# tiborcamargo/KinectPy

Hardware: AMD Instinct MI355X
Metric: Mpoints/sec end-to-end (unproject+filter+ICP), 4-sensor frame (higher is better)
Workload: dtype f64 decisions / f32 storage

## Files before the change

kinectpy_amd/csrc/kpx_icpiter.h:

```cpp
#pragma once
#include "kpx_icpdefs.h"
#include "kpx_fixed.h"
#include "kpx_icpsolve.h"
#include "kpx_nnlocal.h"

namespace kpx {

constexpr int kIRows = kIWaves * kLRows;
constexpr int kCertHist = 64;
constexpr int kChainRec = 32;
constexpr int kChainRecords = 64;
constexpr int kChainWords = 24;
constexpr unsigned long long kChainEmpty = 0xFFF8C0DEC0DEC0DEull;
constexpr int kAccSet = kAccCopies * kAcc * kFixedWords;
constexpr int kStampBlocks = 4096;
__device__ unsigned long long g_icp_stamp[kStampBlocks][8];
__device__ unsigned long long g_icp_wave[kStampBlocks * 4][4];
__device__ unsigned long long g_cert_check[8];
__device__ unsigned long long g_chain_stamp[64][48];
__device__ __forceinline__ void chain_tick(unsigned long long *row, int slot, bool on)
{
    if (row && on) row[slot] = wall_clock64();
}
__device__ __forceinline__ void phase_tick(unsigned long long *__restrict__ armed, int slot, unsigned bid)
{
    if (!armed || threadIdx.x || bid >= kStampBlocks) return;
    __builtin_nontemporal_store(wall_clock64(), &g_icp_stamp[bid][slot]);
}
__device__ __forceinline__ double cert_skin(bool certs, int k, const IcpState *st, double max_d2, const CertPolicy &pol)
{
    double c_skin = 0.0;
    if (certs && k > 0) {
        const double lm = st->last_motion, md = sqrt(max_d2);
        if (lm <= (double)pol.calm * md) c_skin = fmin(fmax((double)pol.factor * lm, (double)pol.smin * md), (double)pol.smax * md);
    }
    return c_skin;
}
__device__ __forceinline__ bool cert_test(const double s[3], const float src[3], int32_t prev, const float pt[3], int32_t bj, uint32_t cert, const double *Th,
                                          double c_reach, double c_skin, int cert_check, double &rb0)
{
    double d1 = c_reach;
    if (bj != INT_MAX) {
        const double dx = s[0] - (double)pt[0], dy = s[1] - (double)pt[1], dz = s[2] - (double)pt[2];
        d1 = sqrt(fma(dz, dz, fma(dy, dy, dx * dx))) * (1.0 + 1e-12);
    }
    const bool keeps = (prev >= 0) == (bj != INT_MAX);
    const float Lc = __uint_as_float(cert & ~63u);
    double pc[3] = { 0.0, 0.0, 0.0 };
    if (Lc > 0.0f) {
        const double x = src[0], y = src[1], z = src[2];
#pragma unroll
        for (int a = 0; a < 3; ++a) pc[a] = fma(Th[4 * a], x, fma(Th[4 * a + 1], y, fma(Th[4 * a + 2], z, Th[4 * a + 3])));
    }
    const double ex = s[0] - pc[0], ey = s[1] - pc[1], ez = s[2] - pc[2];
    const double moved = sqrt(fma(ez, ez, fma(ey, ey, ex * ex))) * (1.0 + 1e-12);
    const bool certd = Lc > 0.0f && keeps && (d1 + moved) * (1.0 + 1e-6) + 1e-6 < (double)Lc;
    if (certd && !cert_check) rb0 = -1.0;
    else if (c_skin > 0.0) { const double rr = d1 + c_skin; rb0 = fmax(rb0, rr * rr); }
    return certd;
}
__device__ __forceinline__ uint32_t cert_word(unsigned sec, double eps_out, double rb_out, int k)
{
    typedef unsigned uu2 __attribute__((ext_vector_type(2)));
    const uu2 pat = { 0u, sec };
    const double d2nd = sec == 0xFFFFFFFFu ? INFINITY : __builtin_bit_cast(double, pat) - 1.0 - eps_out;
    const double l2 = fmin(rb_out, d2nd);
    const uint32_t lb = l2 > 0.0 && k < kCertHist ? (__float_as_uint(f32_down(sqrt(l2) * (1.0 - 1e-7))) & ~63u) : 0u;
    return lb > 63u ? (lb | (uint32_t)k) : 0u;
}
__device__ __forceinline__ void cert_check_disagreement(int k, int64_t row, int32_t kept, int32_t found, uint32_t word)
{
    if (atomicAdd(&g_cert_check[2], 1ull) == 0ull) {
        g_cert_check[3] = (unsigned long long)k; g_cert_check[4] = (unsigned long long)row;
        g_cert_check[5] = (unsigned long long)(unsigned)kept; g_cert_check[6] = (unsigned long long)(unsigned)found;
        g_cert_check[7] = (unsigned long long)(word & ~63u);
    }
}
__device__ __forceinline__ void cert_check_count(bool first, int k, const IcpState *st, double c_skin, int certified, int searched)
{
    if (first && g_cert_check[2] == 0ull) {
        g_cert_check[3] = (unsigned long long)k; g_cert_check[4] = __builtin_bit_cast(unsigned long long, st->last_motion);
        g_cert_check[5] = __builtin_bit_cast(unsigned long long, st->motion); g_cert_check[6] = __builtin_bit_cast(unsigned long long, c_skin);
    }
    atomicAdd(&g_cert_check[0], (unsigned long long)certified);
    atomicAdd(&g_cert_check[1], (unsigned long long)searched);
}
__device__ __forceinline__ IcpFuse ticket_fuse(const IcpProblem &P, int max_iter, double rel_fit, double rel_rmse, unsigned long long tag, int light,
                                               CertPolicy pol, double *chain_rec, unsigned long long *stamp)
{
    return IcpFuse{ (IcpState *)nullptr, P.ring, max_iter, rel_fit, rel_rmse, P.result, P.progress, tag, P.ring + kAccSet,
                    (light & 1) ? P.light_key : (double *)nullptr, P.sbbox, (light & 2) ? P.cert : (uint32_t *)nullptr,
                    (light & 2) ? P.thist : (double *)nullptr, (light & 4) ? 1 : 0, pol, chain_rec, stamp };
}
template <int THREADS, bool SEARCHED>
__device__ __forceinline__ unsigned long long winner_take(unsigned long long *acc, unsigned long long *ticket, bool plane, double *s_sums, int tix_w)
{
    if (tix_w < kAcc) s_sums[tix_w] = acc_live(plane, tix_w) ? fixed_total_coherent(acc, tix_w) : 0.0;
    const unsigned long long n_searched = SEARCHED ? searched_take(ticket, tix_w) : 0ull;
    if (THREADS > 64) __syncthreads(); else wave_lds_fence();
    for (int e = tix_w; e < kAccSet; e += THREADS) __hip_atomic_store(acc + e, 0ull, __ATOMIC_RELAXED, __HIP_MEMORY_SCOPE_AGENT);
    if (tix_w == 0) __hip_atomic_store(ticket, 0ull, __ATOMIC_RELAXED, __HIP_MEMORY_SCOPE_AGENT);
    return n_searched;
}
__device__ __forceinline__ void winner_publish(IcpState *st, const IcpState *work, double *thist, int k, unsigned long long *progress, unsigned long long tag,
                                               unsigned long long n_searched, int64_t n, int lane)
{
    if (lane < (int)(sizeof(IcpState) / sizeof(double))) reinterpret_cast<double *>(st)[lane] = reinterpret_cast<const double *>(work)[lane];
    if (thist && k + 1 < kCertHist && lane < 12) thist[12 * (k + 1) + lane] = work->T[lane];
    if (lane == 0 && progress)
        __hip_atomic_store(progress, tag | progress_searched(n_searched, n) | ((unsigned long long)(work->done ? 1 : 0) << 32) | (unsigned long long)(unsigned)(k + 1),
                           __ATOMIC_RELAXED, __HIP_MEMORY_SCOPE_SYSTEM);
}

template <bool PERSIST = false>
__device__ __forceinline__ void icp_iter_body(const unsigned bid, const unsigned nblocks, const float *__restrict__ src, int64_t n, const float *__restrict__ tgt,
                                                       const float *__restrict__ tn, const double *__restrict__ Bs,
                                                       const int32_t *__restrict__ orig, const float *__restrict__ tile_box,
                                                       const float *__restrict__ group_box, int32_t n_groups,
                                                       const double *__restrict__ tbbox, const int32_t *__restrict__ row_of,
                                                       const float *__restrict__ src_sorted, int32_t *__restrict__ idx_sorted,
                                                       float *__restrict__ ptgt_sorted,
                                                       int32_t *__restrict__ idx_cur, double *__restrict__ d2_cur, double max_d2, int mode,
                                                       int k, const IcpState *__restrict__ st, unsigned long long *acc,
                                                       unsigned long long *__restrict__ tile_visits, IcpFuse fuse)
{
    const unsigned tix = PERSIST ? (unsigned)opaque_i((int)threadIdx.x) : threadIdx.x;
    __shared__ IcpState s_state;
    __shared__ double s_sums[kAcc];
    __shared__ float rowk[kIWaves][16][8];
    __shared__ float rowsrc[kIWaves][16][3];
    __shared__ uint32_t rowc[kIWaves][16];
    __shared__ int32_t rowi[kIWaves][16][2];
    __shared__ double s_key;
    const int wave = PERSIST ? __builtin_amdgcn_readfirstlane((int)(tix >> 6)) : (int)(tix >> 6), lane = tix & 63, q = lane >> 4, j = lane & 15;
    const int64_t row_base = ((int64_t)bid * kIWaves + wave) * kLRows;
    const int64_t last = n - 1;
    const unsigned long long t_block_start = (tile_visits && tix == 0) ? wall_clock64() : 0ull;
    const double t2max = target_t2max(tbbox);
    float my_src[3] = { 0.0f, 0.0f, 0.0f }, my_pt[3] = { 0.0f, 0.0f, 0.0f }, my_nrm[3] = { 0.0f, 0.0f, 0.0f };
    int32_t my_row = 0, my_prev = -1;
    uint32_t my_cert = 0u;
    const bool certs = fuse.ticket && fuse.light_key && fuse.cert;
    if (PERSIST && k > 0) {
        if (lane < 16) {
            my_row = rowi[wave][lane][1];
#pragma unroll
            for (int a = 0; a < 3; ++a) { my_src[a] = rowsrc[wave][lane][a]; my_pt[a] = rowk[wave][lane][a]; my_nrm[a] = rowk[wave][lane][3 + a]; }
            my_prev = __float_as_int(rowk[wave][lane][6]);
            if (certs) my_cert = rowc[wave][lane];
        }
    } else if (lane < 16) {
        const int64_t r = row_base + lane < last ? row_base + lane : last;
        if (idx_cur || d2_cur) my_row = row_of[r];
#pragma unroll
        for (int a = 0; a < 3; ++a) my_src[a] = src_sorted[3 * r + a];
        if (PERSIST) {
#pragma unroll
            for (int a = 0; a < 3; ++a) rowsrc[wave][lane][a] = my_src[a];
            rowc[wave][lane] = 0u;
        }
        if (k > 0) {
            my_prev = idx_sorted[r];
#pragma unroll
            for (int a = 0; a < 3; ++a) my_pt[a] = ptgt_sorted[3 * r + a];
            if (certs) my_cert = fuse.cert[r];
        }
    }
    __shared__ double s_thist[kCertHist][12];
    if (PERSIST) {
        if (certs && k < kCertHist && tix < 12) s_thist[k][tix] = st->T[tix];
    } else if (certs && k > 0)
        for (int e = tix; e < 12 * (k < kCertHist ? k : kCertHist); e += kIThreads) (&s_thist[0][0])[e] = fuse.thist[e];
    GroupPre gpre;
    group_pre_load(gpre, group_box, n_groups, lane);
    if (!PERSIST && mode == 1 && k > 0 && lane < 16) {
        const float *np_ = tn + 3 * (int64_t)(my_prev > 0 ? my_prev : 0);
#pragma unroll
        for (int a = 0; a < 3; ++a) my_nrm[a] = np_[a];
    }
    const double *Tk = st->T;
    static_assert(sizeof(IcpState) % sizeof(double) == 0, "IcpState is copied as doubles");
    if (fuse.ticket && tix < sizeof(IcpState) / sizeof(double))
        reinterpret_cast<double *>(&s_state)[tix] = reinterpret_cast<const double *>(st)[tix];
    if (fuse.pair) {
        const IcpState *in = fuse.pair + ((k + 1) & 1);
        IcpState *out = fuse.pair + (k & 1);
        const unsigned long long *prev = fuse.ring + (int64_t)((k + 2) % 3) * kAccSet;
        if (k > 0 && tix < kAcc) s_sums[tix] = acc_live(mode == 1, (int)tix) ? fixed_total(prev, tix) : 0.0;
        if (tix == 0) s_state = *in;
        __syncthreads();
        if (s_state.done) {
            if (bid == 0 && tix == 0) *out = s_state;
            return;
        }
        __shared__ FinishScratch s_fs;
        if (k > 0 && wave == 0)
            icp_finish_wave(s_sums, n, mode, k - 1, fuse.max_iter, fuse.rel_fit, fuse.rel_rmse, &s_state, bid == 0 ? fuse.result : (double *)nullptr,
                            s_fs, lane);
        __syncthreads();
        if (bid == 0) {
            unsigned long long *next = fuse.ring + (int64_t)((k + 1) % 3) * kAccSet;
            for (int e = tix; e < kAccSet; e += kIThreads) next[e] = 0ull;
            if (tix == 0) {
                *out = s_state;
                if (k > 0 && fuse.progress)
                    __hip_atomic_store(fuse.progress, fuse.tag | ((unsigned long long)(s_state.done ? 1 : 0) << 32) | (unsigned long long)(unsigned)k,
                                       __ATOMIC_RELEASE, __HIP_MEMORY_SCOPE_SYSTEM);
            }
        }
        if (s_state.done) return;
        Tk = s_state.T;
        acc = fuse.ring + (int64_t)(k % 3) * kAccSet;
    } else if (st->done) return;
    bool skip = false;
    if (fuse.ticket && fuse.light_key) {
        const double key = PERSIST ? (k > 0 ? s_key : 0.0) : fuse.light_key[bid];
        skip = key > 0.0 && (st->motion + st->reach) * (1.0 + 1e-6) + 1e-6 < key;
    }
    __shared__ double s_light[kIWaves];
    const int nacc = mode == 1 ? kAcc : 17;
    if (tile_visits && tix == 0 && bid < kStampBlocks) { g_icp_stamp[bid][7] = skip ? 1ull : 0ull; g_icp_stamp[bid][6] = (unsigned long long)nblocks; }
    do {
    if (skip) break;
    __shared__ int32_t lists[kIWaves][kLScratch];
    __shared__ double rowd[kIWaves][16][kRowStride];
    __shared__ float rowf[kIWaves][16][kRowFStride];
    __shared__ double sh[kAcc][kIRows + 1];
    if (tile_visits && tix == 0 && bid < kStampBlocks) {
        g_icp_stamp[bid][0] = t_block_start;
        g_icp_stamp[bid][6] = (unsigned long long)nblocks;
    }
    phase_tick(tile_visits, 1, bid);
    if (certs && (k > 0 || PERSIST)) __syncthreads();
    if (PERSIST && fuse.stamp && tix == 0) {
        const unsigned long long t = wall_clock64();
        if (bid == 0) fuse.stamp[0] = t;
        atomicMax(&fuse.stamp[5], t);
        atomicMin(&fuse.stamp[10], t);
    }

    const double c_reach = certs ? st->reach : 0.0;
    const double c_skin = cert_skin(certs, k, st, max_d2, fuse.pol);
    bool my_active = true, my_certd = false;
    if (lane < 16) {
        const int64_t i = my_row;
        double s[3];
        xform_row(Tk, my_src, s);
        const double seed = row_seed(s);
        double bv = INFINITY;
        int32_t bj = INT_MAX;
        if (k > 0 && my_prev >= 0) { bv = partner_bound(s, seed, my_pt); bj = my_prev; }
        bound_clamp(seed, max_d2, t2max, bv, bj);
        double rb0 = bv - 1.0;
        if (certs) {
            const bool certd = cert_test(s, my_src, my_prev, my_pt, bj, my_cert, s_thist[my_cert & 63u], c_reach, c_skin, fuse.cert_check, rb0);
            my_active = (!certd || fuse.cert_check) && row_base + lane <= last;
            my_certd = certd && row_base + lane <= last;
        }
        rowd[wave][lane][0] = s[0]; rowd[wave][lane][1] = s[1]; rowd[wave][lane][2] = s[2];
        rowd[wave][lane][3] = rb0;
        rowd[wave][lane][4] = seed; rowd[wave][lane][5] = bv;
        rowi[wave][lane][0] = bj; rowi[wave][lane][1] = (int32_t)i;
#pragma unroll
        for (int a = 0; a < 3; ++a) { rowk[wave][lane][a] = my_pt[a]; rowk[wave][lane][3 + a] = my_nrm[a]; }
        rowk[wave][lane][6] = __int_as_float(my_prev);
    }
    if (PERSIST && fuse.stamp) {
        const bool searched = lane < 16 && my_active && !my_certd;
        const unsigned long long sm = __builtin_amdgcn_ballot_w64(searched);
        const unsigned long long np = __builtin_amdgcn_ballot_w64(searched && my_prev < 0);
        const unsigned long long nc = __builtin_amdgcn_ballot_w64(searched && (my_cert & ~63u) == 0u);
        if (lane == 0 && sm) {
            atomicAdd(&fuse.stamp[26], 1ull); atomicAdd(&fuse.stamp[27], (unsigned long long)__builtin_popcountll(sm));
            atomicAdd(&fuse.stamp[28], (unsigned long long)__builtin_popcountll(np)); atomicAdd(&fuse.stamp[29], (unsigned long long)__builtin_popcountll(nc));
        }
    }
    const unsigned act_mask = (unsigned)(__builtin_amdgcn_ballot_w64(lane < 16 && my_active) & 0xFFFFull);
    const unsigned certd_mask = (unsigned)(__builtin_amdgcn_ballot_w64(lane < 16 && my_certd) & 0xFFFFull);
    wave_lds_fence();
    WaveRows w;
    w.a = q < 3 ? rowd[wave][j][q] : 1.0;
    w.rows = &rowd[wave][0][0];
    w.rowsf = &rowf[wave][0][0];
#pragma unroll
    for (int r = 0; r < 4; ++r) {
        const int rr = q + 4 * r;
        w.seed[r] = rowd[wave][rr][4];
        w.best[r] = rowd[wave][rr][5];
        w.bcol[r] = rowi[wave][rr][0];
        w.rb0[r] = rowd[wave][rr][3];
    }
    w.skin = c_skin;
    w.act_mask = act_mask;
    w.light_gap2 = -1.0;
    w.dbg = (PERSIST && fuse.stamp && bid == 0 && wave == 0) ? fuse.stamp + 16 : (unsigned long long *)nullptr;
    phase_tick(tile_visits, 2, bid);
    if (PERSIST) chain_tick(fuse.stamp, 1, bid == 0 && tix == 0);
    const unsigned long long t_sweep = tile_visits ? wall_clock64() : 0ull;
    unsigned long long swept = 0ull;
    int lane_p = 0, wave_p = 0, q_p = 0, j_p = 0;
    int64_t row_base_p = 0;
    auto rederive = [&]() {
        lane_p = opaque_i((int)(threadIdx.x & 63)); wave_p = opaque_i((int)(threadIdx.x >> 6)); q_p = lane_p >> 4; j_p = lane_p & 15;
        row_base_p = ((int64_t)bid * kIWaves + wave_p) * kLRows;
    };
    if (act_mask != 0u) {
        wave_lds_fence();
        swept = sweep_wave<true, true, PERSIST>(w, Bs, orig, tile_box, group_box, n_groups, t2max, lists[wave], &gpre);
        rederive();
        if (certs && fuse.cert_check && j_p == 0) {
#pragma unroll
            for (int r = 0; r < 4; ++r) {
                const int rr = q_p + 4 * r;
                if (((certd_mask >> rr) & 1u) != 0u && w.bcol[r] != rowi[wave_p][rr][0])
                    cert_check_disagreement(k, row_base_p + rr, rowi[wave_p][rr][0], w.bcol[r], PERSIST ? rowc[wave_p][rr] : fuse.cert[row_base_p + rr]);
            }
        }
        if (certs && j_p == 0) {
#pragma unroll
            for (int r = 0; r < 4; ++r) {
                const int rr = q_p + 4 * r;
                if (((act_mask >> rr) & 1u) != 0u && ((certd_mask >> rr) & 1u) == 0u) {
                    const uint32_t cw = cert_word(w.sec[r], w.eps_out, w.rb_out[r], k);
                    if (PERSIST) rowc[wave_p][rr] = cw; else fuse.cert[row_base_p + rr] = cw;
                }
            }
        }
    }
    if (act_mask == 0u) rederive();
    __shared__ int s_cnt[kIWaves];
    if (lane_p == 0) s_cnt[wave_p] = __builtin_popcount(act_mask & ~certd_mask);
    const unsigned visited = (unsigned)(swept & 0xFFFFu);
    if (certs && fuse.cert_check && lane_p == 0)
        cert_check_count(bid == 0 && wave_p == 0, k, st, c_skin, __builtin_popcount(certd_mask), __builtin_popcount(act_mask & ~certd_mask));
    if (lane_p == 0) s_light[wave_p] = act_mask == 0xFFFFu ? w.light_gap2 : -1.0;
    if (tile_visits && lane_p == 0 && bid < kStampBlocks && kIWaves <= 4) {
        unsigned long long *o = g_icp_wave[bid * 4 + wave_p];
        int with = 0;
#pragma unroll
        for (int r = 0; r < 4; ++r) with += (w.bcol[r] >= 0 && w.bcol[r] != INT_MAX) ? 1 : 0;
        o[0] = t_sweep; o[1] = wall_clock64(); o[2] = swept; o[3] = (unsigned long long)with;
    }
    phase_tick(tile_visits, 3, bid);
    if (PERSIST) chain_tick(fuse.stamp, 2, bid == 0 && lane_p == 0 && wave_p == 0);
    if (PERSIST && fuse.stamp && bid == 0 && lane_p == 0 && wave_p == 0) { fuse.stamp[13] = swept; fuse.stamp[14] = (unsigned long long)act_mask | ((unsigned long long)certd_mask << 16); }
    if (tile_visits && lane_p == 0) atomicAdd(tile_visits + ((bid * kIWaves + wave_p) & (kVisitSlots - 1)), (unsigned long long)visited);
    wave_lds_fence();
    if (j_p == 0) {
#pragma unroll
        for (int r = 0; r < 4; ++r) rowi[wave_p][q_p + 4 * r][0] = w.bcol[r];
    }
    wave_lds_fence();

    const int lane_e = lane_p, wave_e = wave_p;
    if (lane_e < 16) {
        const int col = wave_e * 16 + lane_e;
        sh[0][col] = 0.0; sh[1][col] = 0.0;
        for (int a = acc_lo(mode == 1); a < nacc; ++a) sh[a][col] = 0.0;
        if (row_base_p + lane_e <= last) {
            const int32_t bj = rowi[wave_e][lane_e][0];
            const int64_t i = rowi[wave_e][lane_e][1];
            const bool none = bj < 0 || bj == INT_MAX;
            const int32_t out_j = none ? -1 : bj;
            const int32_t prev_j = __float_as_int(rowk[wave_e][lane_e][6]);
            const bool changed = k == 0 || out_j != prev_j;
            if (idx_cur) idx_cur[i] = out_j;
            if (PERSIST) rowk[wave_e][lane_e][6] = __int_as_float(out_j);
            else if (changed) idx_sorted[row_base_p + lane_e] = out_j;
            if (none) {
                if (d2_cur) d2_cur[i] = INFINITY;
            } else {
                const double s[3] = { rowd[wave_e][lane_e][0], rowd[wave_e][lane_e][1], rowd[wave_e][lane_e][2] };
                float tf[3] = { rowk[wave_e][lane_e][0], rowk[wave_e][lane_e][1], rowk[wave_e][lane_e][2] }, nf[3] = { rowk[wave_e][lane_e][3], rowk[wave_e][lane_e][4], rowk[wave_e][lane_e][5] };
                if (changed) {
                    const float *tp = tgt + 3 * (int64_t)bj;
#pragma unroll
                    for (int c = 0; c < 3; ++c) tf[c] = tp[c];
                    if (mode == 1) {
                        const float *np_ = tn + 3 * (int64_t)bj;
#pragma unroll
                        for (int c = 0; c < 3; ++c) nf[c] = np_[c];
                    }
#pragma unroll
                    for (int c = 0; c < 3; ++c) {
                        if (PERSIST) { rowk[wave_e][lane_e][c] = tf[c]; rowk[wave_e][lane_e][3 + c] = nf[c]; }
                        else ptgt_sorted[3 * (row_base_p + lane_e) + c] = tf[c];
                    }
                }
                const double t[3] = { (double)tf[0], (double)tf[1], (double)tf[2] };
                const double d2 = pair_d2(s, t);
                if (d2_cur) d2_cur[i] = d2;
                if (d2 < max_d2) pair_terms(s, t, d2, mode != 1, mode == 1, nf, [&](int slot, double v) { sh[slot][col] = v; });
            }
        }
    }
    __syncthreads();
    phase_tick(tile_visits, 4, bid);
    const int tix_e = wave_e * 64 + lane_e;
    if (tix_e < nacc && acc_live(mode == 1, tix_e)) {
        unsigned long long lo = 0ull, hi = 0ull;
#pragma unroll
        for (int t = 0; t < kIWaves; ++t) {
            unsigned long long l, h;
            fixed_split(tile_tree16(&sh[tix_e][16 * t]), l, h);
            fixed_accumulate(lo, hi, l, h);
        }
        unsigned long long *slot = acc + (((int64_t)(bid & (kAccCopies - 1)) * kAcc + tix_e) * kFixedWords);
        if (fuse.ticket) fixed_add_words_performed(slot, lo, hi); else fixed_add_words(slot, lo, hi);
    } else if (!PERSIST && fuse.ticket && tix_e == nacc) {
        int cnt = 0;
#pragma unroll
        for (int wv = 0; wv < kIWaves; ++wv) cnt += s_cnt[wv];
        if (cnt) {
            const unsigned long long back = __hip_atomic_fetch_add(fuse.ticket + kSearchedWord + (bid & 7u), (unsigned long long)cnt, __ATOMIC_RELAXED, __HIP_MEMORY_SCOPE_AGENT);
            asm volatile("" ::"v"(back));
        }
    }
    if (fuse.light_key && tix == kIThreads - 1) {
        double g2 = INFINITY;
        bool light = true;
#pragma unroll
        for (int wv = 0; wv < kIWaves; ++wv) { light = light && s_light[wv] >= 0.0; g2 = fmin(g2, s_light[wv]); }
        const double nk = light ? st->motion + sqrt(g2) * (1.0 - 1e-9) : 0.0;
        if (PERSIST) s_key = nk; else fuse.light_key[bid] = nk;
    }
    phase_tick(tile_visits, 5, bid);
    } while (false);
    if (PERSIST && fuse.stamp && tix == 0) {
        const unsigned long long t = wall_clock64();
        if (bid == 0) fuse.stamp[3] = t;
        atomicMax(&fuse.stamp[11], t);
    }
    if (!fuse.ticket) return;
    __shared__ unsigned s_ticket;
    __syncthreads();
    if (tix == 0) s_ticket = (unsigned)__hip_atomic_fetch_add(fuse.ticket, 1ull, __ATOMIC_RELAXED, __HIP_MEMORY_SCOPE_AGENT);
    __syncthreads();
    if (PERSIST && fuse.stamp && tix == 0) {
        const unsigned long long t = wall_clock64();
        if (bid == 0) fuse.stamp[4] = t;
        atomicMax(&fuse.stamp[6], t);
    }
    if (s_ticket != nblocks - 1u) return;
    __builtin_amdgcn_fence(__ATOMIC_ACQUIRE, "agent");
    const int tix_w = opaque_i((int)threadIdx.x);
    const unsigned long long n_searched = winner_take<kIThreads, !PERSIST>(acc, fuse.ticket, mode == 1, s_sums, tix_w);
    if (PERSIST) chain_tick(fuse.stamp, 7, tix == 0);
    if (PERSIST) asm volatile("s_waitcnt vmcnt(0)" ::: "memory");
    if (wave != 0) {
        if (PERSIST) __syncthreads();
        return;
    }
    __shared__ FinishScratch s_tail;
    const double *tbbox_w = tbbox;
    asm volatile("" : "+s"(tbbox_w));
    const double t2max_w = target_t2max(tbbox_w);
    IcpState *stw = const_cast<IcpState *>(st);
    IcpState *work = &s_state;
    if (PERSIST)
        icp_finish_wave_call(s_sums, n, mode, k, fuse.max_iter, fuse.rel_fit, fuse.rel_rmse, work, (double *)nullptr, &s_tail, lane,
                             fuse.light_key ? fuse.sbbox : (const double *)nullptr, max_d2, t2max_w, fuse.stamp ? fuse.stamp + 32 : (unsigned long long *)nullptr);
    else
        icp_finish_wave(s_sums, n, mode, k, fuse.max_iter, fuse.rel_fit, fuse.rel_rmse, work, fuse.result, s_tail, lane,
                        LightSkip{ fuse.light_key ? fuse.sbbox : (const double *)nullptr, max_d2, t2max_w });
    wave_lds_fence();
    if (PERSIST) chain_tick(fuse.stamp, 8, lane == 0);
    if (PERSIST) {
        static_assert(sizeof(IcpState) == kChainWords * sizeof(double), "record layout");
        __syncthreads();
        if (lane < kChainWords)
            __hip_atomic_store(reinterpret_cast<unsigned long long *>(fuse.chain_rec + (size_t)kChainRec * (k + 1)) + lane,
                               reinterpret_cast<const unsigned long long *>(&s_state)[lane], __ATOMIC_RELAXED, __HIP_MEMORY_SCOPE_AGENT);
        if (work->done && fuse.result) {
            if (lane < 16) fuse.result[lane] = work->T[lane];
            if (lane == 0) { fuse.result[16] = work->fitness; fuse.result[17] = work->rmse; fuse.result[18] = (double)k; fuse.result[19] = work->count; }
        }
        if (lane == 0 && fuse.progress && work->done)
            __hip_atomic_store(fuse.progress, fuse.tag | (1ull << 32) | (unsigned long long)(unsigned)(k + 1), __ATOMIC_RELAXED, __HIP_MEMORY_SCOPE_SYSTEM);
        chain_tick(fuse.stamp, 9, lane == 0);
        if (fuse.stamp && lane == 0) fuse.stamp[12] = __builtin_amdgcn_s_memtime();
        return;
    }
    winner_publish(stw, work, fuse.cert ? fuse.thist : (double *)nullptr, k, fuse.progress, fuse.tag, n_searched, n, lane);
}


__global__ __launch_bounds__(kIThreads) __attribute__((amdgpu_waves_per_eu(KPX_ICP_WPE, KPX_ICP_WPE))) void icp_iter_kernel(const float *__restrict__ src, int64_t n, const float *__restrict__ tgt,
                                                       const float *__restrict__ tn, const double *__restrict__ Bs,
                                                       const int32_t *__restrict__ orig, const float *__restrict__ tile_box,
                                                       const float *__restrict__ group_box, int32_t n_groups,
                                                       const double *__restrict__ tbbox, const int32_t *__restrict__ row_of,
                                                       const float *__restrict__ src_sorted, int32_t *__restrict__ idx_sorted,
                                                       float *__restrict__ ptgt_sorted,
                                                       int32_t *__restrict__ idx_cur, double *__restrict__ d2_cur, double max_d2, int mode,
                                                       int k, const IcpState *__restrict__ st, unsigned long long *acc,
                                                       unsigned long long *__restrict__ tile_visits, IcpFuse fuse)
{
    icp_iter_body(blockIdx.x, gridDim.x, src, n, tgt, tn, Bs, orig, tile_box, group_box, n_groups, tbbox, row_of, src_sorted, idx_sorted, ptgt_sorted,
                  idx_cur, d2_cur, max_d2, mode, k, st, acc, tile_visits, fuse);
}

__global__ __launch_bounds__(kIThreads) __attribute__((amdgpu_waves_per_eu(KPX_ICP_WPE, KPX_ICP_WPE))) void icp_iter_batch_kernel(IcpBatchArgs args, double max_d2, int mode, int max_iter, double rel_fit,
                                                       double rel_rmse, unsigned long long *__restrict__ tile_visits, int light, CertPolicy pol)
{
    const IcpProblem &P = args.p[batch_problem(args)];
    const unsigned bid = blockIdx.x - P.block0;
    const float *__restrict__ tgt = P.tgt, *__restrict__ tn = P.tn, *__restrict__ tile_box = P.tile_box, *__restrict__ group_box = P.group_box;
    const double *__restrict__ Bs = P.Bs, *__restrict__ tbbox = P.tbbox;
    const int32_t *__restrict__ orig = P.orig;
    const int32_t n_groups = P.n_groups;
    const int k = P.k;
    const IcpFuse fuse = ticket_fuse(P, max_iter, rel_fit, rel_rmse, P.tag, light, pol, nullptr, nullptr);
    icp_iter_body(bid, P.blocks, P.src, P.n, tgt, tn, Bs, orig, tile_box, group_box, n_groups, tbbox, P.row_of, P.src_sorted, P.idx_sorted, P.ptgt_sorted,
                  P.idx_cur, P.d2_cur, max_d2, mode, k, P.pair, P.ring, tile_visits, fuse);
}

__global__ __launch_bounds__(kIThreads) __attribute__((amdgpu_waves_per_eu(KPX_ICP_WPE, KPX_ICP_WPE))) void icp_chain_kernel(IcpBatchArgs args, const float *__restrict__ tgt,
                                                       const float *__restrict__ tn, const double *__restrict__ Bs,
                                                       const int32_t *__restrict__ orig, const float *__restrict__ tile_box,
                                                       const float *__restrict__ group_box, int32_t n_groups,
                                                       const double *__restrict__ tbbox, double max_d2, int mode, int max_iter, double rel_fit,
                                                       double rel_rmse, unsigned long long tag, unsigned long long *__restrict__ tile_visits, int light,
                                                       CertPolicy pol, unsigned long long limit_ticks, unsigned long long *abort_word)
{
    const int pi = batch_problem(args);
    const IcpProblem &P = args.p[pi];
    const unsigned bid = blockIdx.x - P.block0;
    __shared__ IcpState s_cur;
    __shared__ int s_abort;
    const unsigned long long t0 = wall_clock64();
    if (threadIdx.x == 0) s_abort = 0;
    __syncthreads();
    for (int k = 0; k <= max_iter; ++k) {
        asm volatile("" : "+s"(tgt), "+s"(tn), "+s"(Bs), "+s"(orig), "+s"(tile_box), "+s"(group_box), "+s"(tbbox));
        asm volatile("" : "+s"(max_d2), "+s"(mode), "+s"(n_groups), "+s"(pol.calm), "+s"(pol.factor), "+s"(pol.smin), "+s"(pol.smax));
        const IcpFuse fuse = ticket_fuse(P, max_iter, rel_fit, rel_rmse, tag, light, pol, P.chain_rec,
                                         ((light & 8) && pi == 0 && k < 64) ? &g_chain_stamp[k][0] : (unsigned long long *)nullptr);
        if (threadIdx.x < kChainWords) {
            const unsigned long long *w = reinterpret_cast<const unsigned long long *>(P.chain_rec + (size_t)kChainRec * k) + threadIdx.x;
            unsigned long long v = __hip_atomic_load(w, __ATOMIC_RELAXED, __HIP_MEMORY_SCOPE_AGENT);
            unsigned spins = 0;
            while (v == kChainEmpty) {
                __builtin_amdgcn_s_sleep(2);
                if ((++spins & 255u) == 0u && wall_clock64() - t0 > limit_ticks) { s_abort = 1; break; }
                v = __hip_atomic_load(w, __ATOMIC_RELAXED, __HIP_MEMORY_SCOPE_AGENT);
            }
            reinterpret_cast<unsigned long long *>(&s_cur)[threadIdx.x] = v;
        }
        __syncthreads();
        if (s_abort) {
            if (threadIdx.x == 0) __hip_atomic_store(abort_word, tag | 1ull, __ATOMIC_RELAXED, __HIP_MEMORY_SCOPE_SYSTEM);
            if (P.result && threadIdx.x < 20) P.result[threadIdx.x] = __builtin_nan("");
            return;
        }
        if (s_cur.done) break;
        icp_iter_body<true>(bid, P.blocks, P.src, P.n, tgt, tn, Bs, orig, tile_box, group_box, n_groups, tbbox, P.row_of, P.src_sorted, P.idx_sorted, P.ptgt_sorted,
                            P.idx_cur, P.d2_cur, max_d2, mode, k, &s_cur, P.ring, tile_visits, fuse);
        __syncthreads();
    }
}

__global__ __launch_bounds__(256) void icp_batch_init_kernel(IcpBatchArgs args, Mat16x8 T0)
{
    const int pi = batch_problem(args);
    const IcpProblem &P = args.p[pi];
    const unsigned bid = blockIdx.x - P.block0;
    const int c = threadIdx.x & 3;
    for (int rr = threadIdx.x >> 2; rr < kIRows; rr += 64) {
        const int64_t r = (int64_t)bid * kIRows + rr;
        if (r < P.n && c < 3) P.src_sorted[3 * r + c] = P.src[3 * (int64_t)P.row_of[r] + c];
    }
    if (threadIdx.x == 0) P.light_key[bid] = 0.0;
    if (bid == 0) {
        for (int e = threadIdx.x; e < 3 * kAccSet; e += 256) P.ring[e] = 0ull;
        if (threadIdx.x >= 64 && threadIdx.x < 76) P.thist[threadIdx.x - 64] = T0.m[pi][threadIdx.x - 64];
        if (P.chain_rec) {
            unsigned long long *rw = reinterpret_cast<unsigned long long *>(P.chain_rec);
            for (int e = kChainRec + threadIdx.x; e < kChainRecords * kChainRec; e += 256) rw[e] = kChainEmpty;
            IcpState *r0 = reinterpret_cast<IcpState *>(P.chain_rec);
            if (threadIdx.x >= 128 && threadIdx.x < 144) r0->T[threadIdx.x - 128] = T0.m[pi][threadIdx.x - 128];
            if (threadIdx.x == 144) state_fresh(r0);
        }
        if (threadIdx.x < 32) {
            IcpState *st = P.pair + (threadIdx.x >> 4);
            st->T[threadIdx.x & 15] = T0.m[pi][threadIdx.x & 15];
            if ((threadIdx.x & 15) == 0) state_fresh(st);
        }
    }
}

}
```

Measured before the change: 2786.

## Use last-arriving wave for block reduction and single-wave ticket finish in non-persistent ICP

In the non-persistent ICP iteration kernel, the block-wide barrier before the per-tile accumulator reduction is replaced by an LDS arrival counter. Only the last wave to arrive reduces the packed shared accumulator rows into the global fixed-point slots; the other waves exit early. The shared accumulator is compacted into a dense row layout that skips unused slots. The grid-wide ticket and finish step now runs in one wave instead of the whole block. This is meant to cut barrier stalls and shared-memory footprint, but it relies on correct LDS fencing between waves and adds an extra barrier at block start.

```diff
diff --git a/kinectpy_amd/csrc/kpx_icpiter.h b/kinectpy_amd/csrc/kpx_icpiter.h
--- a/kinectpy_amd/csrc/kpx_icpiter.h
+++ b/kinectpy_amd/csrc/kpx_icpiter.h
@@ -27,6 +27,17 @@
     if (!armed || threadIdx.x || bid >= kStampBlocks) return;
     __builtin_nontemporal_store(wall_clock64(), &g_icp_stamp[bid][slot]);
 }
+__device__ __forceinline__ void phase_tick_wave(unsigned long long *__restrict__ armed, int slot, unsigned bid, int lane)
+{
+    if (!armed || lane || bid >= kStampBlocks) return;
+    __builtin_nontemporal_store(wall_clock64(), &g_icp_stamp[bid][slot]);
+}
+constexpr int kAccDense = 2 + (kAcc - 17);
+static_assert(kAccDense >= 17, "the point-to-point slots 0..16 fit");
+__host__ __device__ constexpr int acc_dense(int slot) { return slot < 17 ? slot : slot - 15; }
+__host__ __device__ constexpr int acc_dense_live(bool plane) { return plane ? kAccDense : 17; }
+__host__ __device__ constexpr int acc_dense_slot(bool plane, int row) { return row < 2 ? row : row - 2 + acc_lo(plane); }
+static_assert(acc_dense(acc_dense_slot(true, 28)) == 28 && acc_dense(acc_dense_slot(false, 16)) == 16 && acc_dense_slot(true, 2) == 17, "dense rows <-> slots");
 __device__ __forceinline__ double cert_skin(bool certs, int k, const IcpState *st, double max_d2, const CertPolicy &pol)
 {
     double c_skin = 0.0;
@@ -220,18 +231,25 @@
     __shared__ double s_light[kIWaves];
     const int nacc = mode == 1 ? kAcc : 17;
     if (tile_visits && tix == 0 && bid < kStampBlocks) { g_icp_stamp[bid][7] = skip ? 1ull : 0ull; g_icp_stamp[bid][6] = (unsigned long long)nblocks; }
+    __shared__ unsigned s_arrive;
     do {
-    if (skip) break;
+    if (skip) {
+        if (!PERSIST && wave != 0) return;
+        break;
+    }
     __shared__ int32_t lists[kIWaves][kLScratch];
     __shared__ double rowd[kIWaves][16][kRowStride];
     __shared__ float rowf[kIWaves][16][kRowFStride];
-    __shared__ double sh[kAcc][kIRows + 1];
+    constexpr int kShRows = PERSIST ? kAcc : kAccDense;
+    __shared__ double sh[kShRows][kIRows + 1];
+    auto sh_row = [](int slot) { return PERSIST ? slot : acc_dense(slot); };
     if (tile_visits && tix == 0 && bid < kStampBlocks) {
         g_icp_stamp[bid][0] = t_block_start;
         g_icp_stamp[bid][6] = (unsigned long long)nblocks;
     }
     phase_tick(tile_visits, 1, bid);
-    if (certs && (k > 0 || PERSIST)) __syncthreads();
+    if (!PERSIST && kIWaves > 1 && tix == 0) s_arrive = 0u;
+    if ((!PERSIST && kIWaves > 1) || (certs && (k > 0 || PERSIST))) __syncthreads();
     if (PERSIST && fuse.stamp && tix == 0) {
         const unsigned long long t = wall_clock64();
         if (bid == 0) fuse.stamp[0] = t;
@@ -355,8 +373,11 @@
     const int lane_e = lane_p, wave_e = wave_p;
     if (lane_e < 16) {
         const int col = wave_e * 16 + lane_e;
-        sh[0][col] = 0.0; sh[1][col] = 0.0;
-        for (int a = acc_lo(mode == 1); a < nacc; ++a) sh[a][col] = 0.0;
+        if (PERSIST) {
+            sh[0][col] = 0.0; sh[1][col] = 0.0;
+            for (int a = acc_lo(mode == 1); a < nacc; ++a) sh[a][col] = 0.0;
+        } else
+            for (int a = 0; a < acc_dense_live(mode == 1); ++a) sh[a][col] = 0.0;
         if (row_base_p + lane_e <= last) {
             const int32_t bj = rowi[wave_e][lane_e][0];
             const int64_t i = rowi[wave_e][lane_e][1];
@@ -390,10 +411,49 @@
                 const double t[3] = { (double)tf[0], (double)tf[1], (double)tf[2] };
                 const double d2 = pair_d2(s, t);
                 if (d2_cur) d2_cur[i] = d2;
-                if (d2 < max_d2) pair_terms(s, t, d2, mode != 1, mode == 1, nf, [&](int slot, double v) { sh[slot][col] = v; });
+                if (d2 < max_d2) pair_terms(s, t, d2, mode != 1, mode == 1, nf, [&](int slot, double v) { sh[sh_row(slot)][col] = v; });
             }
         }
     }
+    if constexpr (!PERSIST) {
+        if (kIWaves > 1) {
+            wave_lds_fence();
+            unsigned arrived = 0u;
+            if (lane_e == 0) arrived = __hip_atomic_fetch_add(&s_arrive, 1u, __ATOMIC_RELAXED, __HIP_MEMORY_SCOPE_WORKGROUP);
+            if (__builtin_amdgcn_readfirstlane((int)arrived) != kIWaves - 1) return;
+            wave_lds_fence();
+        }
+        phase_tick_wave(tile_visits, 4, bid, lane_e);
+        const bool plane = mode == 1;
+        if (lane_e < acc_dense_live(plane)) {
+            const int slot_e = acc_dense_slot(plane, lane_e);
+            unsigned long long lo = 0ull, hi = 0ull;
+#pragma unroll
+            for (int t = 0; t < kIWaves; ++t) {
+                unsigned long long l, h;
+                fixed_split(tile_tree16(&sh[lane_e][16 * t]), l, h);
+                fixed_accumulate(lo, hi, l, h);
+            }
+            unsigned long long *slot = acc + (((int64_t)(bid & (kAccCopies - 1)) * kAcc + slot_e) * kFixedWords);
+            if (fuse.ticket) fixed_add_words_performed(slot, lo, hi); else fixed_add_words(slot, lo, hi);
+        } else if (fuse.ticket && lane_e == nacc) {
+            int cnt = 0;
+#pragma unroll
+            for (int wv = 0; wv < kIWaves; ++wv) cnt += s_cnt[wv];
+            if (cnt) {
+                const unsigned long long back = __hip_atomic_fetch_add(fuse.ticket + kSearchedWord + (bid & 7u), (unsigned long long)cnt, __ATOMIC_RELAXED, __HIP_MEMORY_SCOPE_AGENT);
+                asm volatile("" ::"v"(back));
+            }
+        }
+        if (fuse.light_key && lane_e == 63) {
+            double g2 = INFINITY;
+            bool light = true;
+#pragma unroll
+            for (int wv = 0; wv < kIWaves; ++wv) { light = light && s_light[wv] >= 0.0; g2 = fmin(g2, s_light[wv]); }
+            fuse.light_key[bid] = light ? st->motion + sqrt(g2) * (1.0 - 1e-9) : 0.0;
+        }
+        phase_tick_wave(tile_visits, 5, bid, lane_e);
+    } else {
     __syncthreads();
     phase_tick(tile_visits, 4, bid);
     const int tix_e = wave_e * 64 + lane_e;
@@ -407,14 +467,6 @@
         }
         unsigned long long *slot = acc + (((int64_t)(bid & (kAccCopies - 1)) * kAcc + tix_e) * kFixedWords);
         if (fuse.ticket) fixed_add_words_performed(slot, lo, hi); else fixed_add_words(slot, lo, hi);
-    } else if (!PERSIST && fuse.ticket && tix_e == nacc) {
-        int cnt = 0;
-#pragma unroll
-        for (int wv = 0; wv < kIWaves; ++wv) cnt += s_cnt[wv];
-        if (cnt) {
-            const unsigned long long back = __hip_atomic_fetch_add(fuse.ticket + kSearchedWord + (bid & 7u), (unsigned long long)cnt, __ATOMIC_RELAXED, __HIP_MEMORY_SCOPE_AGENT);
-            asm volatile("" ::"v"(back));
-        }
     }
     if (fuse.light_key && tix == kIThreads - 1) {
         double g2 = INFINITY;
@@ -422,10 +474,32 @@
 #pragma unroll
         for (int wv = 0; wv < kIWaves; ++wv) { light = light && s_light[wv] >= 0.0; g2 = fmin(g2, s_light[wv]); }
         const double nk = light ? st->motion + sqrt(g2) * (1.0 - 1e-9) : 0.0;
-        if (PERSIST) s_key = nk; else fuse.light_key[bid] = nk;
+        s_key = nk;
     }
     phase_tick(tile_visits, 5, bid);
+    }
     } while (false);
+    if constexpr (!PERSIST) {
+        if (!fuse.ticket) return;
+        asm volatile("s_waitcnt vmcnt(0)" ::: "memory");
+        wave_lds_fence();
+        const int lane_w = opaque_i((int)(threadIdx.x & 63));
+        unsigned tk = 0u;
+        if (lane_w == 0) tk = (unsigned)__hip_atomic_fetch_add(fuse.ticket, 1ull, __ATOMIC_RELAXED, __HIP_MEMORY_SCOPE_AGENT);
+        tk = (unsigned)__builtin_amdgcn_readfirstlane((int)tk);
+        wave_lds_fence();
+        if (tk != nblocks - 1u) return;
+        __builtin_amdgcn_fence(__ATOMIC_ACQUIRE, "agent");
+        const unsigned long long n_searched = winner_take<64, true>(acc, fuse.ticket, mode == 1, s_sums, lane_w);
+        __shared__ FinishScratch s_tail;
+        const double *tbbox_w = tbbox;
+        asm volatile("" : "+s"(tbbox_w));
+        const double t2max_w = target_t2max(tbbox_w);
+        icp_finish_wave(s_sums, n, mode, k, fuse.max_iter, fuse.rel_fit, fuse.rel_rmse, &s_state, fuse.result, s_tail, lane_w,
+                        LightSkip{ fuse.light_key ? fuse.sbbox : (const double *)nullptr, max_d2, t2max_w });
+        wave_lds_fence();
+        winner_publish(const_cast<IcpState *>(st), &s_state, fuse.cert ? fuse.thist : (double *)nullptr, k, fuse.progress, fuse.tag, n_searched, n, lane_w);
+    } else {
     if (PERSIST && fuse.stamp && tix == 0) {
         const unsigned long long t = wall_clock64();
         if (bid == 0) fuse.stamp[3] = t;
@@ -444,28 +518,23 @@
     if (s_ticket != nblocks - 1u) return;
     __builtin_amdgcn_fence(__ATOMIC_ACQUIRE, "agent");
     const int tix_w = opaque_i((int)threadIdx.x);
-    const unsigned long long n_searched = winner_take<kIThreads, !PERSIST>(acc, fuse.ticket, mode == 1, s_sums, tix_w);
-    if (PERSIST) chain_tick(fuse.stamp, 7, tix == 0);
-    if (PERSIST) asm volatile("s_waitcnt vmcnt(0)" ::: "memory");
+    winner_take<kIThreads, false>(acc, fuse.ticket, mode == 1, s_sums, tix_w);
+    chain_tick(fuse.stamp, 7, tix == 0);
+    asm volatile("s_waitcnt vmcnt(0)" ::: "memory");
     if (wave != 0) {
-        if (PERSIST) __syncthreads();
+        __syncthreads();
         return;
     }
     __shared__ FinishScratch s_tail;
     const double *tbbox_w = tbbox;
     asm volatile("" : "+s"(tbbox_w));
     const double t2max_w = target_t2max(tbbox_w);
-    IcpState *stw = const_cast<IcpState *>(st);
     IcpState *work = &s_state;
-    if (PERSIST)
-        icp_finish_wave_call(s_sums, n, mode, k, fuse.max_iter, fuse.rel_fit, fuse.rel_rmse, work, (double *)nullptr, &s_tail, lane,
-                             fuse.light_key ? fuse.sbbox : (const double *)nullptr, max_d2, t2max_w, fuse.stamp ? fuse.stamp + 32 : (unsigned long long *)nullptr);
-    else
-        icp_finish_wave(s_sums, n, mode, k, fuse.max_iter, fuse.rel_fit, fuse.rel_rmse, work, fuse.result, s_tail, lane,
-                        LightSkip{ fuse.light_key ? fuse.sbbox : (const double *)nullptr, max_d2, t2max_w });
+    icp_finish_wave_call(s_sums, n, mode, k, fuse.max_iter, fuse.rel_fit, fuse.rel_rmse, work, (double *)nullptr, &s_tail, lane,
+                         fuse.light_key ? fuse.sbbox : (const double *)nullptr, max_d2, t2max_w, fuse.stamp ? fuse.stamp + 32 : (unsigned long long *)nullptr);
     wave_lds_fence();
-    if (PERSIST) chain_tick(fuse.stamp, 8, lane == 0);
-    if (PERSIST) {
+    chain_tick(fuse.stamp, 8, lane == 0);
+    {
         static_assert(sizeof(IcpState) == kChainWords * sizeof(double), "record layout");
         __syncthreads();
         if (lane < kChainWords)
@@ -479,9 +548,8 @@
             __hip_atomic_store(fuse.progress, fuse.tag | (1ull << 32) | (unsigned long long)(unsigned)(k + 1), __ATOMIC_RELAXED, __HIP_MEMORY_SCOPE_SYSTEM);
         chain_tick(fuse.stamp, 9, lane == 0);
         if (fuse.stamp && lane == 0) fuse.stamp[12] = __builtin_amdgcn_s_memtime();
-        return;
-    }
-    winner_publish(stw, work, fuse.cert ? fuse.thist : (double *)nullptr, k, fuse.progress, fuse.tag, n_searched, n, lane);
+    }
+    }
 }
 
 
```

After: 2820, median of 6. +1.2%, better.
